# zhongzisha/multi_frame_super_resolution

Hardware: AMD Instinct MI355X
Metric: Mpix/s end-to-end (N-frame burst -> x2 SR) (higher is better)
Workload: dtype f32

## Files before the change

multi_frame_super_resolution_amd/csrc/accumulate_fast.hip:

```cpp
#include <cstdlib>

#include "accumulate_common.hpp"
#include <type_traits>

namespace {

template <int CFA>
struct Cfa {
    static constexpr int col(int yp, int xp) { return (CFA >> (2 * ((yp << 1) | xp))) & 3; }
    static constexpr int pos_of(int c)
    {
        int n = 0, p = -1;
        for (int a = 0; a < 4; a++)
            if (((CFA >> (2 * a)) & 3) == c) {
                n++;
                p = a;
            }
        return n == 1 ? p : -1;
    }
    static constexpr int count(int c)
    {
        int n = 0;
        for (int a = 0; a < 4; a++)
            if (((CFA >> (2 * a)) & 3) == c) n++;
// ... 75 lines not shown
            chS[2] = at_pos(S, pb >> 1, pb & 1);
            chW[2] = at_pos(W, pb >> 1, pb & 1);
        }
        chS[1] = (totS - chS[0]) - chS[2];
        chW[1] = (totW - chW[0]) - chW[2];
    }
#pragma unroll
    for (int c = 0; c < 3; c++) {
        accP[3 * K + c] = __builtin_fmaf(__builtin_fmaf(-lv.black[c], chW[c], chS[c]), lv.invWhite[c], accP[3 * K + c]);
        accW[3 * K + c] += chW[c];
    }
}

__device__ __forceinline__ void tap_weights13(float kx, float ky, float kz, float (&w)[13])
{
    const float a1 = kx * -0.72134752044448170368f, b1 = ky * -0.72134752044448170368f;
    const float c1 = kz * -0.72134752044448170368f;
    const float A[3] = {0.0f, a1, 4.0f * a1}, B[3] = {0.0f, b1, 4.0f * b1};
#pragma unroll
    for (int n = 0; n < 12; n++) {
        const int py = n / 5 - 2, px = n % 5 - 2;
        const int apx = px < 0 ? -px : px, apy = py < 0 ? -py : py;
        const float d = apx == 0 ? B[apy] : (apy == 0 ? A[apx] : A[apx] + B[apy]);
        w[n] = __builtin_amdgcn_exp2f(px * py == 0 ? d : d + (float)(2 * px * py) * c1);
    }
    w[12] = 1.0f;
}

template <int K, int CFA>
__device__ __forceinline__ void strip_pixel_sites(const float (&C)[5][3], const float (&s)[3][3], uint32_t mby, uint32_t nby, uint32_t mP,
                                                   uint32_t mQ, const StripLevels& lv, float* accP, float* accW)
{
    auto andm = [](uint32_t m, float a) { return __uint_as_float(m & __float_as_uint(a)); };
    float Om[3][3];
#pragma unroll
    for (int i = 0; i < 3; i++) {
        Om[0][i] = C[0][i] + andm(nby, C[1][i]);
        Om[1][i] = C[2][i] + selm(mby, C[1][i], C[3][i]);
        Om[2][i] = andm(mby, C[3][i]) + C[4][i];
    }
    float S[2][2], W[2][2];
    S[0][0] = __builtin_fmaf(s[2][2], Om[2][2], __builtin_fmaf(s[2][0], Om[2][0], __builtin_fmaf(s[0][2], Om[0][2], s[0][0] * Om[0][0])));
    W[0][0] = (Om[0][0] + Om[0][2]) + (Om[2][0] + Om[2][2]);
    S[0][1] = __builtin_fmaf(s[2][1], Om[2][1], s[0][1] * Om[0][1]);
    W[0][1] = Om[0][1] + Om[2][1];
    S[1][0] = __builtin_fmaf(s[1][2], Om[1][2], s[1][0] * Om[1][0]);
    W[1][0] = Om[1][0] + Om[1][2];
    S[1][1] = s[1][1] * Om[1][1];
    W[1][1] = Om[1][1];

    classes_to_channels<K, CFA>(S, W, mP, mQ, lv, accP, accW);
}

template <int K, int CFA, bool PARITY = false, typename RawF, typename MaskF>
__device__ __forceinline__ void strip_pixel_w(int X, int Y, int sx, int sy, const float (&w)[13], RawF rawf, MaskF mval,
                                               const StripLevels& lv, float* accP, float* accW)
{
    const int qx = X + sx - 2, qy = Y + sy - 2;
    const int x0 = qx >> 1, y0 = qy >> 1;
    uint32_t mbx = 0u - (uint32_t)(qx & 1), mby = 0u - (uint32_t)(qy & 1);
    uint32_t nbx = ~mbx, nby = ~mby;
    asm volatile("" : "+v"(mbx), "+v"(nbx), "+v"(mby), "+v"(nby));
    const uint32_t mP = 0u - (uint32_t)(x0 & 1), mQ = 0u - (uint32_t)(y0 & 1);
    auto andm = [](uint32_t m, float a) { return __uint_as_float(m & __float_as_uint(a)); };

    float s[3][3];
    rawf(x0, y0, s);

    float wl[13], wh[13];
#pragma unroll
    for (int n = 0; n < 13; n++) {
        const int it = n % 5;
        if (it == 1 || it == 3) {
            wl[n] = andm(nbx, w[n]);
            wh[n] = andm(mbx, w[n]);
        }
    }
    auto W_ = [&](int jt, int it) { const int n = jt * 5 + it; return w[n <= 12 ? n : 24 - n]; };
    auto WL = [&](int jt, int it) { const int n = jt * 5 + it; return wl[n <= 12 ? n : 24 - n]; };
    auto WH = [&](int jt, int it) { const int n = jt * 5 + it; return wh[n <= 12 ? n : 24 - n]; };

    const uint32_t mY13 = mQ ^ mby;
    constexpr int cellLo = (K + 0 + 2) >> 2;
    auto cidx = [](int it) { return (((K + it + 2) >> 2) == ((K + 2) >> 2)) ? 0 : 1; };

    float C[5][3];
#pragma unroll
    for (int jt = 0; jt < 5; jt++) {
        uint32_t mya;
        if (jt == 0 || jt == 4) mya = mQ;
        if (jt == 2) mya = ~mQ;
        if (jt == 1) mya = mY13;
        if (jt == 3) mya = ~mY13;
        float Ee[2], Eo[2];
        if constexpr (PARITY) {
            const int eQ = ((qy << 2) & 8) | ((qx + qx) & 4);
            const int by2 = (qy << 3) & 8;
            const int e = (jt == 0 || jt == 4) ? eQ : (jt == 2 ? (eQ ^ 8) : (jt == 1 ? (eQ ^ by2) : (eQ ^ 8 ^ by2)));
#pragma unroll
            for (int c = 0; c < 2; c++) {
                Ee[c] = mval(jt, cellLo + c, e);
                Eo[c] = mval(jt, cellLo + c, e ^ 4);
            }
        } else {
#pragma unroll
            for (int c = 0; c < 2; c++) {
                float m[3];
#pragma unroll
                for (int ch = 0; ch < 3; ch++) m[ch] = mval(jt, cellLo + c, ch);
                resolve_certainty<CFA>(mya, mP, m, Ee[c], Eo[c]);
            }
        }
        C[jt][0] = cidx(0) == cidx(1) ? (W_(jt, 0) + WL(jt, 1)) * Ee[cidx(0)]
                                      : __builtin_fmaf(WL(jt, 1), Ee[cidx(1)], W_(jt, 0) * Ee[cidx(0)]);
        {
            float acc;
            if (cidx(1) == cidx(2))
                acc = (WH(jt, 1) + W_(jt, 2)) * Eo[cidx(1)];
            else
                acc = __builtin_fmaf(W_(jt, 2), Eo[cidx(2)], WH(jt, 1) * Eo[cidx(1)]);
            if (cidx(3) == cidx(1) && cidx(1) == cidx(2))
                acc = ((WH(jt, 1) + W_(jt, 2)) + WL(jt, 3)) * Eo[cidx(1)];
            else
                acc = __builtin_fmaf(WL(jt, 3), Eo[cidx(3)], acc);
            C[jt][1] = acc;
        }
        C[jt][2] = cidx(3) == cidx(4) ? (WH(jt, 3) + W_(jt, 4)) * Ee[cidx(3)]
                                      : __builtin_fmaf(W_(jt, 4), Ee[cidx(4)], WH(jt, 3) * Ee[cidx(3)]);
    }
    strip_pixel_sites<K, CFA>(C, s, mby, nby, mP, mQ, lv, accP, accW);
}

template <int K, int CFA, typename RawF>
__device__ __forceinline__ void strip_pixel_sat(int X, int Y, int sx, int sy, const float (&w)[13], const float (&P)[3][4], RawF rawf,
                                                 const StripLevels& lv, float* accP, float* accW)
{
    const int qx = X + sx - 2, qy = Y + sy - 2;
    const int x0 = qx >> 1, y0 = qy >> 1;
    uint32_t mbx = 0u - (uint32_t)(qx & 1), mby = 0u - (uint32_t)(qy & 1);
    uint32_t nby = ~mby;
    asm volatile("" : "+v"(mbx), "+v"(mby), "+v"(nby));
    const uint32_t mP = 0u - (uint32_t)(x0 & 1), mQ = 0u - (uint32_t)(y0 & 1);
    float s[3][3];
    rawf(x0, y0, s);
    auto W_ = [&](int jt, int it) { const int n = jt * 5 + it; return w[n <= 12 ? n : 24 - n]; };
    auto P_ = [&](int jt, int i) { return jt <= 2 ? P[jt][i] : P[4 - jt][3 - i]; };
    float C[5][3];
#pragma unroll
    for (int jt = 0; jt < 5; jt++) {
        C[jt][0] = selm(mbx, W_(jt, 0), P_(jt, 0));
        C[jt][1] = selm(mbx, P_(jt, 1), P_(jt, 2));
        C[jt][2] = selm(mbx, P_(jt, 3), W_(jt, 4));
    }
    strip_pixel_sites<K, CFA>(C, s, mby, nby, mP, mQ, lv, accP, accW);
}

__device__ __forceinline__ void tap_pair_sums(const float (&w)[13], float (&P)[3][4])
{
    auto W_ = [&](int jt, int it) { const int n = jt * 5 + it; return w[n <= 12 ? n : 24 - n]; };
#pragma unroll
    for (int r = 0; r < 3; r++)
#pragma unroll
        for (int i = 0; i < 4; i++) P[r][i] = W_(r, i) + W_(r, i + 1);
}

template <int K, int CFA, bool PARITY = false, typename MaskF>
__device__ __forceinline__ void strip_pixel(int X, int Y, int sx, int sy, float kx, float ky, float kz,
                                             const uint16_t* __restrict__ raw, int dimX, MaskF mval,
                                             const StripLevels& lv, float* accP, float* accW)
{
    float w[13];
    tap_weights13(kx, ky, kz, w);
    auto rawf = [&](int x0, int y0, float (&s)[3][3]) {
        const uint16_t* r = raw + (size_t)y0 * dimX + x0;
#pragma unroll
        for (int j = 0; j < 3; j++)
#pragma unroll
            for (int i = 0; i < 3; i++) s[j][i] = (float)r[j * dimX + i];
    };
    strip_pixel_w<K, CFA, PARITY>(X, Y, sx, sy, w, rawf, mval, lv, accP, accW);
}

#define STRIP_MARGIN 16
#ifndef MARGIN_TAP_SUMS
#define MARGIN_TAP_SUMS 1
#endif

template <int SCALE, bool WIN = false>
__global__ void __launch_bounds__(256)
    k_accumulateMargin(const uint16_t* __restrict__ raw, pix3* __restrict__ imgOut, pix3* __restrict__ totalWeights,
                       const float4* __restrict__ certaintyMask, mfsr_tex2d kernelParam, mfsr_tex2d shifts, Levels3 glv,
                       int dimX, int dimY, int strideOut, int strideMask, int cfaPacked, int rowBegin, int rowEnd, MarginRects mr)
{
    constexpr int scale = SCALE;
    if constexpr (WIN) {
        int x, y;
        if (!margin_rect_pixel(mr, blockIdx.x * blockDim.x + threadIdx.x, x, y)) return;
        accumulate_pixel_generic<GEOM_FULL, true, MARGIN_TAP_SUMS>(x, y, raw, imgOut, totalWeights, certaintyMask, kernelParam, shifts,
                                                                   glv, dimX, dimY, scale, strideOut, strideMask, cfaPacked,
                                                                   mr.accX0, mr.accY0);
        return;
    }
    const int hrW = scale * dimX, hrH = scale * dimY, M = STRIP_MARGIN;
    const int rowLen = hrW - 2;
    const int nTop = (M - 1) * rowLen;
    const int nBot = (M - 1) * rowLen;
    const int sideLen = 2 * (M - 1);
    const int nSide = (hrH - 2 * M) * sideLen;
    const int idx = blockIdx.x * blockDim.x + threadIdx.x;
    int x, y;
    if (idx < nTop) {
        y = 1 + idx / rowLen;
        x = 1 + idx % rowLen;
    } else if (idx < nTop + nBot) {
        const int r = idx - nTop;
        y = hrH - M + r / rowLen;
        x = 1 + r % rowLen;
    } else if (idx < nTop + nBot + nSide) {
        const int r = idx - nTop - nBot;
        y = M + r / sideLen;
        const int c = r % sideLen;
        x = c < M - 1 ? 1 + c : hrW - M + (c - (M - 1));
    } else {
        return;
    }
    if (y < rowBegin || y >= rowEnd) return;
    accumulate_pixel_generic<GEOM_FULL, true, MARGIN_TAP_SUMS>(x, y, raw, imgOut, totalWeights, certaintyMask, kernelParam, shifts, glv, dimX,
                                              dimY, scale, strideOut, strideMask, cfaPacked);
}

struct TileFrame {
    const uint16_t* raw;
    const float4* mask;
// ... 195 lines not shown
    const int Y = (blockIdx.y + rowBlock0) * 4 + threadIdx.y;
    const int hrW = 2 * dimX, hrH = 2 * dimY;
    const int X0 = 4 * tx;
    if (X0 < STRIP_MARGIN || X0 >= hrW - STRIP_MARGIN || Y < STRIP_MARGIN || Y >= hrH - STRIP_MARGIN) return;
    if (WIN && (X0 < wx0 || X0 >= wx1)) return;

    const size_t accOff = WIN ? (size_t)(Y - wy0) * strideOut + (size_t)(X0 - wx0) * 12 : (size_t)Y * strideOut + (size_t)X0 * 12;
    float4* pP = (float4*)((char*)imgOut + accOff);
    float4* pW = (float4*)((char*)totalWeights + accOff);
    float accP[12], accW[12];
    {
        const float4 a0 = pP[0], a1 = pP[1], a2 = pP[2];
        const float4 b0 = pW[0], b1 = pW[1], b2 = pW[2];
        accP[0] = a0.x; accP[1] = a0.y; accP[2] = a0.z; accP[3] = a0.w;
        accP[4] = a1.x; accP[5] = a1.y; accP[6] = a1.z; accP[7] = a1.w;
        accP[8] = a2.x; accP[9] = a2.y; accP[10] = a2.z; accP[11] = a2.w;
        accW[0] = b0.x; accW[1] = b0.y; accW[2] = b0.z; accW[3] = b0.w;
        accW[4] = b1.x; accW[5] = b1.y; accW[6] = b1.z; accW[7] = b1.w;
        accW[8] = b2.x; accW[9] = b2.y; accW[10] = b2.z; accW[11] = b2.w;
    }
#pragma unroll
    for (int n = 0; n < NF; n++)
        strip_frame<CFA, FR>(tx, Y, X0, fr.f[n].raw, fr.f[n].mask, kernelParam, fr.f[n].shifts, glv, lv, dimX, dimY, strideMask,
                             cfaPacked, accP, accW);
    pP[0] = make_float4(accP[0], accP[1], accP[2], accP[3]);
    pP[1] = make_float4(accP[4], accP[5], accP[6], accP[7]);
    pP[2] = make_float4(accP[8], accP[9], accP[10], accP[11]);
    pW[0] = make_float4(accW[0], accW[1], accW[2], accW[3]);
    pW[1] = make_float4(accW[4], accW[5], accW[6], accW[7]);
    pW[2] = make_float4(accW[8], accW[9], accW[10], accW[11]);
}

#define TILE_COLS 66
#ifndef TILE_WAVES
#define TILE_WAVES 4
#endif
#ifndef TILE_WAVES2
#define TILE_WAVES2 4
#endif
#ifndef TILE_GROUP_BOTH_PLANES
#define TILE_GROUP_BOTH_PLANES 1
#endif
#define TILE_WAVES_NF(NF) ((NF) == 1 ? TILE_WAVES : ((NF) > 2 && TILE_GROUP_BOTH_PLANES) ? (TILE_LDS_ALIAS_ON ? 4 : 3) : TILE_WAVES2)
#ifndef TILE_PIXEL_MAJOR
#define TILE_PIXEL_MAJOR 1
#endif
#define TILE_LDS_ALIAS_ON (TILE_LDS_ALIAS && TILE_PIXEL_MAJOR && TILE_GROUP_BOTH_PLANES)
#ifndef TILE_LDS_ALIAS
#define TILE_LDS_ALIAS 1
#endif
#ifndef TILE_SAT_PATH
#define TILE_SAT_PATH 1
#endif

template <int CFA, int NF, int FR = 4, bool WIN = false>
__global__ void __launch_bounds__(256, (FR != 4 ? 3 : TILE_WAVES_NF(NF)))
    k_accumulate2xTile(TileFrames<NF> fr, pix3* __restrict__ imgOut, pix3* __restrict__ totalWeights, mfsr_tex2d kernelParam,
                       Levels3 glv, StripLevels lv, int dimX, int dimY, int strideOut, int strideMask, int cfaPacked,
                       int tilesX, int tilesY, int tilesPerXcd, int fresh, int tileY0, int tileX0, int wx0, int wx1, int wy0)
{
    const int pid = (int)blockIdx.x;
    const int tile = tilesPerXcd > 0 ? (pid & 7) * tilesPerXcd + (pid >> 3) : pid;
    if (tile >= tilesX * tilesY) return;
    const int bIdYrel = tile / tilesX, bIdX = tile - bIdYrel * tilesX + (WIN ? tileX0 : 0);
    const int bIdY = bIdYrel + tileY0;
    static_assert(FR == 4 || FR == 2, "field resolution");
    constexpr int FC = 256 / FR + 2, FROWS = 4 / FR + 2;
    constexpr int PL = (NF <= 2 || TILE_GROUP_BOTH_PLANES) ? 2 : 1;
    constexpr bool ALIAS = TILE_LDS_ALIAS_ON && FR == 4 && NF > 2 && PL == 2;
    __shared__ __attribute__((aligned(16))) float4 sAcc[PL][4][192];
    __shared__ float4 sKown[ALIAS ? 1 : FROWS][ALIAS ? 1 : FC];
    __shared__ float2 sFown[ALIAS ? 1 : NF][ALIAS ? 1 : FROWS][ALIAS ? 1 : FC];
    static_assert(!ALIAS || sizeof(float4) * FROWS * FC + sizeof(float2) * NF * FROWS * FC <= sizeof(float4) * 4 * 192, "field texels fit a plane-set");
    float4(*sK)[FC] = ALIAS ? (float4(*)[FC]) & sAcc[PL - 1][0][0] : (float4(*)[FC]) & sKown[0][0];
    float2(*sF)[FROWS][FC] = ALIAS ? (float2(*)[FROWS][FC])((char*)&sAcc[PL - 1][0][0] + sizeof(float4) * FROWS * FC)
                                   : (float2(*)[FROWS][FC]) & sFown[0][0][0];
    __shared__ float4 sM[NF][3][TILE_COLS];
    __shared__ uint32_t sUnsat[3][TILE_COLS];
    __shared__ __attribute__((aligned(16))) float sColA[256];
    __shared__ float sRowB[4];
    const int lx = threadIdx.x, ly = threadIdx.y;
    const int tx = bIdX * 64 + lx;
    const int Y = bIdY * 4 + ly;
    const int hrW = 2 * dimX, hrH = 2 * dimY;
    const int X0 = 4 * tx;
    const int fw = kernelParam.width, fh = kernelParam.height;
    const int mw = dimX / 2, mh = dimY / 2;
    {
        const int t = ly * 64 + lx;
        if constexpr (FR != 4) {
            for (int i = t; i < FROWS * FC; i += 256) {
                const int r = i / FC, c = i - r * FC;
                const int gy = bIdY * (4 / FR) - 1 + r, gx = bIdX * (256 / FR) - 1 + c;
                const int fy = clampi(gy, 0, fh - 1), fx = clampi(gx, 0, fw - 1);
                float4 k = row_ptr((const float4*)kernelParam.ptr, kernelParam.pitch, fy)[fx];
                k.w = psd_ok(k.x, k.y, k.z) ? 1.0f : 0.0f;
                sK[r][c] = k;
#pragma unroll
                for (int n = 0; n < NF; n++) sF[n][r][c] = row_ptr((const float2*)fr.f[n].shifts.ptr, fr.f[n].shifts.pitch, fy)[fx];
            }
            if (t < 3 * TILE_COLS) {
                const int r = t / TILE_COLS, c = t - r * TILE_COLS;
                const int gy = bIdY - 1 + r, gx = bIdX * 64 - 1 + c;
                uint32_t unsat = 0;
#pragma unroll
                for (int n = 0; n < NF; n++) {
                    const float4 m = row_ptr(fr.f[n].mask, strideMask, clampi(gy, 0, mh - 1))[clampi(gx, 0, mw - 1)];
                    const float mc[3] = {sane(m.x), sane(m.y), sane(m.z)};
                    sM[n][r][c] = make_float4(mc[Cfa<CFA>::col(0, 0)], mc[Cfa<CFA>::col(0, 1)], mc[Cfa<CFA>::col(1, 0)],
                                              mc[Cfa<CFA>::col(1, 1)]);
                    if (!(mc[0] == 1.0f && mc[1] == 1.0f && mc[2] == 1.0f)) unsat |= 1u << n;
                }
                sUnsat[r][c] = unsat;
            }
        } else if (t < 3 * TILE_COLS) {
            const int r = t / TILE_COLS, c = t - r * TILE_COLS;
            const int gy = bIdY - 1 + r, gx = bIdX * 64 - 1 + c;
            const int fy = clampi(gy, 0, fh - 1), fx = clampi(gx, 0, fw - 1);
            float4 k = row_ptr((const float4*)kernelParam.ptr, kernelParam.pitch, fy)[fx];
            k.w = psd_ok(k.x, k.y, k.z) ? 1.0f : 0.0f;
            sK[r][c] = k;
            uint32_t unsat = 0;
#pragma unroll
            for (int n = 0; n < NF; n++) {
                sF[n][r][c] = row_ptr((const float2*)fr.f[n].shifts.ptr, fr.f[n].shifts.pitch, fy)[fx];
                const float4 m = row_ptr(fr.f[n].mask, strideMask, clampi(gy, 0, mh - 1))[clampi(gx, 0, mw - 1)];
                const float mc[3] = {sane(m.x), sane(m.y), sane(m.z)};
                sM[n][r][c] = make_float4(mc[Cfa<CFA>::col(0, 0)], mc[Cfa<CFA>::col(0, 1)], mc[Cfa<CFA>::col(1, 0)],
                                          mc[Cfa<CFA>::col(1, 1)]);
                if (!(mc[0] == 1.0f && mc[1] == 1.0f && mc[2] == 1.0f)) unsat |= 1u << n;
            }
            sUnsat[r][c] = unsat;
        }
        {
            const int X = bIdX * 256 + t;
            const float posX = ((float)X + 0.5f) / (float)hrW;
            float xB = posX * (float)fw - 0.5f;
            if (!finitef(xB)) xB = 0.0f;
            const float fxf = floorf(xB);
            const int txc = FR == 4 ? X >> 2 : X >> 1, ci = FR == 4 ? ((t & 3) < 2 ? 0 : 1) : (t & 1);
            const bool ok = (f2i(fxf) == txc - 1 + ci) && (txc + ci <= fw - 1);
            sColA[t] = ok ? xB - fxf : -1.0f;
        }
        if (t < 4) {
            const int Yr = bIdY * 4 + t;
            const float posY = ((float)Yr + 0.5f) / (float)hrH;
            float yB = posY * (float)fh - 0.5f;
            if (!finitef(yB)) yB = 0.0f;
            const float fyf = floorf(yB);
            const int frr = FR == 4 ? (t < 2 ? 0 : 1) : (t + 1) >> 1;
            const bool ok = (f2i(fyf) == bIdY * (4 / FR) - 1 + frr) && f2i(fyf) >= 0 && f2i(fyf) + 1 <= fh - 1;
            sRowB[t] = ok ? yB - fyf : -1.0f;
        }
    }
    const bool rowLive = Y >= STRIP_MARGIN && Y < hrH - STRIP_MARGIN;
    const size_t rowBytes = (size_t)hrW * 12;
    const size_t segByte = (size_t)bIdX * 3072;
    const size_t winB0 = WIN ? (size_t)wx0 * 12 : 0, winB1 = WIN ? (size_t)wx1 * 12 : 0;
    char* gP = WIN ? (char*)imgOut + (size_t)(Y - wy0) * strideOut : (char*)imgOut + (size_t)Y * strideOut + segByte;
    char* gW = WIN ? (char*)totalWeights + (size_t)(Y - wy0) * strideOut : (char*)totalWeights + (size_t)Y * strideOut + segByte;
    auto inWin = [&](size_t gb) { return !WIN || (gb >= winB0 && gb + 16 <= winB1); };
    auto chunk = [&](char* g, size_t off) { return WIN ? g + (segByte + off - winB0) : g + off; };
    auto stage_plane = [&](char* g, int pl) {
#pragma unroll
        for (int j = 0; j < 3; j++) {
            if (fresh) {
                sAcc[pl][ly][j * 64 + lx] = make_float4(0.0f, 0.0f, 0.0f, 0.0f);
            } else {
                const size_t off = (size_t)(j * 64 + lx) * 16;
                if (segByte + off + 16 <= rowBytes && inWin(segByte + off))
                    __builtin_amdgcn_global_load_lds((const __attribute__((address_space(1))) void*)chunk(g, off),
                                                     (__attribute__((address_space(3))) void*)&sAcc[pl][ly][j * 64], 16, 0, 0);
            }
        }
    };
    if (rowLive) {
        stage_plane(gP, 0);
        if (PL == 2 && !ALIAS) stage_plane(gW, 1);
    }
    __syncthreads();
    if (!rowLive) return;
    const bool stripLive = X0 >= STRIP_MARGIN && X0 < hrW - STRIP_MARGIN;
// ... 13 lines not shown
        float4 Kt[2][SC];
#pragma unroll
        for (int r = 0; r < 2; r++)
#pragma unroll
            for (int c = 0; c < SC; c++) Kt[r][c] = sK[fr_ + r][cb + c];
        float kAll = ((Kt[0][0].w * Kt[0][1].w) * (Kt[0][2].w * Kt[1][0].w)) * (Kt[1][1].w * Kt[1][2].w);
        if (SC == 4) kAll *= Kt[0][SC - 1].w * Kt[1][SC - 1].w;
        kOk = kAll > 0.0f;
#pragma unroll
        for (int k = 0; k < 4; k++) {
            const int ci = ciOf(k);
            const float w00 = (1.0f - av[k]) * (1.0f - b), w10 = av[k] * (1.0f - b), w01 = (1.0f - av[k]) * b, w11 = av[k] * b;
            auto mix = [&](float t00, float t10, float t01, float t11) {
                return __builtin_fmaf(w11, t11, __builtin_fmaf(w01, t01, __builtin_fmaf(w10, t10, w00 * t00)));
            };
            kxa[k] = mix(Kt[0][ci].x, Kt[0][ci + 1].x, Kt[1][ci].x, Kt[1][ci + 1].x);
            kya[k] = mix(Kt[0][ci].y, Kt[0][ci + 1].y, Kt[1][ci].y, Kt[1][ci + 1].y);
            kza[k] = mix(Kt[0][ci].z, Kt[0][ci + 1].z, Kt[1][ci].z, Kt[1][ci + 1].z);
        }
    }

    float accP[12], accW[12];
#pragma unroll
    for (int i = 0; i < 12; i++) accP[i] = accW[i] = 0.0f;
    const uint32_t xmax = (uint32_t)(2 * dimX - 5), ymax = (uint32_t)(2 * dimY - 5);
    uint32_t safeBits = 0;
    static_assert(NF <= 2 || TILE_PIXEL_MAJOR, "three and four frames per launch exist in pixel-major order only");
#if TILE_PIXEL_MAJOR
    if constexpr (NF > 1 || FR != 4) {
        uint32_t sxy[NF][ALIAS ? 2 : 4];
        int bsx[NF], bsy[NF];
#pragma unroll
        for (int n = 0; n < NF; n++) {
            bsx[n] = bsy[n] = 0;
            if constexpr (ALIAS) {
                sxy[n][0] = sxy[n][1] = 0u;
                const float2 cf = sF[n][1][FC / 2];
                bsx[n] = __builtin_amdgcn_readfirstlane(min(max(round2i(cf.x * 2.0f), -32000), 32000));
                bsy[n] = __builtin_amdgcn_readfirstlane(min(max(round2i(cf.y * 2.0f), -32000), 32000));
            }
            float2 Ft[2][SC];
#pragma unroll
            for (int r = 0; r < 2; r++)
#pragma unroll
                for (int c = 0; c < SC; c++) Ft[r][c] = sF[n][fr_ + r][cb + c];
            bool safe = geomOk && kOk;
#pragma unroll
            for (int k = 0; k < 4; k++) {
                const int ci = ciOf(k);
                const float ux = lerp4(Ft[0][ci].x, Ft[0][ci + 1].x, Ft[1][ci].x, Ft[1][ci + 1].x, av[k], b);
                const float uy = lerp4(Ft[0][ci].y, Ft[0][ci + 1].y, Ft[1][ci].y, Ft[1][ci + 1].y, av[k], b);
                const int sx = round2i(ux * 2.0f), sy = round2i(uy * 2.0f);
                const int qx = X0 + k + sx - 2, qy = Y + sy - 2;
                safe = safe && (uint32_t)(sx + (1 << 15)) < (2u << 15) && (uint32_t)(sy + (1 << 15)) < (2u << 15) &&
                       (uint32_t)qx <= xmax && (uint32_t)qy <= ymax;
                if constexpr (ALIAS) {
                    const int dx = sx - bsx[n], dy = sy - bsy[n];
                    safe = safe && (uint32_t)(dx + 128) < 256u && (uint32_t)(dy + 128) < 256u;
                    sxy[n][0] |= ((uint32_t)dx & 0xffu) << (8 * k);
                    sxy[n][1] |= ((uint32_t)dy & 0xffu) << (8 * k);
                } else {
                    sxy[n][k] = ((uint32_t)sx & 0xffffu) | ((uint32_t)sy << 16);
                }
            }
            if (safe) safeBits |= 1u << n;
        }
        if constexpr (ALIAS) {
            __syncthreads();
            stage_plane(gW, 1);
        }
        const float* mrow[5];
#pragma unroll
        for (int jt = 0; jt < 5; jt++) mrow[jt] = (const float*)&sM[0][((ly + jt - 2) >> 2) + 1][lx];
        const char* rawRow[NF][3];
#pragma unroll
        for (int n = 0; n < NF; n++)
#pragma unroll
            for (int j = 0; j < 3; j++) rawRow[n][j] = (const char*)(fr.f[n].raw + (size_t)j * dimX);
        uint32_t satW = 0;
        if constexpr (TILE_SAT_PATH) {
            const int r0 = ((ly - 2) >> 2) + 1;
            uint32_t u = sUnsat[r0][lx] | sUnsat[r0 + 1][lx];
            if (lx < 2) u |= sUnsat[r0][64 + lx] | sUnsat[r0 + 1][64 + lx];
#pragma unroll
            for (int n = 0; n < NF; n++)
                if (__builtin_amdgcn_ballot_w64((u >> n) & 1u) == 0) satW |= 1u << n;
            satW = (uint32_t)__builtin_amdgcn_readfirstlane((int)satW);
        }
        auto pixel = [&](auto kc) {
            constexpr int k = decltype(kc)::value;
            if (safeBits == 0) return;
            float aP[12];
            aP[3 * k] = aP[3 * k + 1] = aP[3 * k + 2] = 0.0f;
            float w[13];
            tap_weights13(kxa[k], kya[k], kza[k], w);
            float P[3][4];
            if (TILE_SAT_PATH && satW) tap_pair_sums(w, P);
#pragma unroll
            for (int n = 0; n < NF; n++) {
                if ((safeBits >> n) & 1u) {
                    auto rawf = [&](int x0, int y0, float (&sv)[3][3]) {
                        const uint32_t boff = (uint32_t)(y0 * dimX + x0) * 2u;
#pragma unroll
                        for (int j = 0; j < 3; j++) {
                            const char* rb = rawRow[n][j] + (size_t)boff;
#pragma unroll
                            for (int i = 0; i < 3; i++) sv[j][i] = (float)*(const uint16_t*)(rb + 2 * i);
                        }
                    };
                    auto mval = [&](int jt, int cell, int e4) {
                        return *(const float*)((const char*)(mrow[jt] + n * (3 * TILE_COLS * 4) + cell * 4) + e4);
                    };
                    const int sx = ALIAS ? bsx[n] + (int)(int8_t)(sxy[n][0] >> (8 * k)) : (int)(int16_t)(sxy[n][ALIAS ? 0 : k] & 0xffffu);
                    const int sy = ALIAS ? bsy[n] + (int)(int8_t)(sxy[n][1] >> (8 * k)) : (int)sxy[n][ALIAS ? 0 : k] >> 16;
                    if (TILE_SAT_PATH && ((satW >> n) & 1u))
                        strip_pixel_sat<k, CFA>(X0 + k, Y, sx, sy, w, P, rawf, lv, aP, accW);
                    else
                        strip_pixel_w<k, CFA, true>(X0 + k, Y, sx, sy, w, rawf, mval, lv, aP, accW);
                }
            }
            if (k == 0) asm volatile("s_waitcnt vmcnt(0)" ::: "memory");
            float* myP = (float*)&sAcc[0][ly][0] + lx * 12 + 3 * k;
            myP[0] += aP[3 * k];
            myP[1] += aP[3 * k + 1];
            myP[2] += aP[3 * k + 2];
        };
        pixel(std::integral_constant<int, 0>{});
        pixel(std::integral_constant<int, 1>{});
        pixel(std::integral_constant<int, 2>{});
        pixel(std::integral_constant<int, 3>{});
    } else
#endif
    {
#pragma unroll 1
    for (int n = 0; n < NF; n++) {
        const uint16_t* raw = (NF > 1 && n) ? fr.f[NF - 1].raw : fr.f[0].raw;
        float avn[4] = {av[0], av[1], av[2], av[3]};
        float bn = b;
#pragma unroll
        for (int k = 0; k < 4; k++) asm volatile("" : "+v"(avn[k]));
        asm volatile("" : "+v"(bn));
#define av avn
#define b bn
        float2 Ft[2][3];
#pragma unroll
        for (int r = 0; r < 2; r++)
#pragma unroll
            for (int c = 0; c < 3; c++) Ft[r][c] = sF[n][fr_ + r][lx + c];
        int sx[4], sy[4];
        bool safe = geomOk && kOk;
#pragma unroll
        for (int k = 0; k < 4; k++) {
            const int ci = k < 2 ? 0 : 1;
            const float ux = lerp4(Ft[0][ci].x, Ft[0][ci + 1].x, Ft[1][ci].x, Ft[1][ci + 1].x, av[k], b);
            const float uy = lerp4(Ft[0][ci].y, Ft[0][ci + 1].y, Ft[1][ci].y, Ft[1][ci + 1].y, av[k], b);
            sx[k] = round2i(ux * 2.0f);
            sy[k] = round2i(uy * 2.0f);
            const int qx = X0 + k + sx[k] - 2, qy = Y + sy[k] - 2;
            safe = safe && (uint32_t)(sx[k] + (1 << 20)) < (2u << 20) && (uint32_t)(sy[k] + (1 << 20)) < (2u << 20) &&
                   (uint32_t)qx <= xmax && (uint32_t)qy <= ymax;
        }
#undef av
#undef b
        if (safe) {
            safeBits |= 1u << n;
#pragma unroll
            for (int k = 0; k < 4; k++) asm volatile("" : "+v"(kxa[k]), "+v"(kya[k]), "+v"(kza[k]));
            auto mval = [&](int jt, int cell, int e4) {
                const int mr = ((ly + jt - 2) >> 2) + 1;
                return *(const float*)((const char*)&sM[n][mr][lx + cell] + e4);
            };
            strip_pixel<0, CFA, true>(X0 + 0, Y, sx[0], sy[0], kxa[0], kya[0], kza[0], raw, dimX, mval, lv, accP, accW);
            strip_pixel<1, CFA, true>(X0 + 1, Y, sx[1], sy[1], kxa[1], kya[1], kza[1], raw, dimX, mval, lv, accP, accW);
            strip_pixel<2, CFA, true>(X0 + 2, Y, sx[2], sy[2], kxa[2], kya[2], kza[2], raw, dimX, mval, lv, accP, accW);
            strip_pixel<3, CFA, true>(X0 + 3, Y, sx[3], sy[3], kxa[3], kya[3], kza[3], raw, dimX, mval, lv, accP, accW);
        }
    }
    }
    auto add_plane = [&](int pl, const float* acc) {
        float4* my = (float4*)((float*)&sAcc[pl][ly][0] + lx * 12);
#pragma unroll
        for (int j = 0; j < 3; j++) {
            float4 a = my[j];
            a.x += acc[4 * j + 0]; a.y += acc[4 * j + 1]; a.z += acc[4 * j + 2]; a.w += acc[4 * j + 3];
            my[j] = a;
        }
    };
    auto slow_frames = [&](auto doP, auto doW, int plP, int plW) {
        constexpr bool DO_P = decltype(doP)::value, DO_W = decltype(doW)::value;
        float* myP = (float*)&sAcc[plP][ly][0] + lx * 12;
        float* myW = (float*)&sAcc[plW][ly][0] + lx * 12;
#pragma unroll 1
        for (int n = 0; n < NF; n++) {
            if (!((safeBits >> n) & 1u) && stripLive) {
                TileFrame F = fr.f[0];
#pragma unroll
                for (int m = 1; m < NF; m++)
                    if (n == m) F = fr.f[m];
#pragma unroll 1
                for (int k = 0; k < 4; k++) {
                    const int X = X0 + k;
                    if (X >= 1 && X < hrW - 1) {
                        pix3 px = {0.0f, 0.0f, 0.0f}, tw = {0.0f, 0.0f, 0.0f};
                        if (DO_P) px = {myP[3 * k], myP[3 * k + 1], myP[3 * k + 2]};
                        if (DO_W) tw = {myW[3 * k], myW[3 * k + 1], myW[3 * k + 2]};
                        accumulate_pixel_core<GEOM_FULL, true>(X, Y, F.raw, F.mask, kernelParam, F.shifts, glv, dimX, dimY, 2,
                                                               strideMask, cfaPacked, px, tw);
                        if (DO_P) { myP[3 * k] = px.x; myP[3 * k + 1] = px.y; myP[3 * k + 2] = px.z; }
                        if (DO_W) { myW[3 * k] = tw.x; myW[3 * k + 1] = tw.y; myW[3 * k + 2] = tw.z; }
                    }
                }
            }
        }
    };
    auto store_plane = [&](int pl, char* g) {
        asm volatile("s_waitcnt lgkmcnt(0)" ::: "memory");
#pragma unroll
        for (int j = 0; j < 3; j++) {
            const size_t off = (size_t)(j * 64 + lx) * 16;
            const size_t gb = segByte + off;
            const bool sideMargin = gb < (size_t)STRIP_MARGIN * 12 || gb + 16 > rowBytes - (size_t)STRIP_MARGIN * 12;
            if (gb + 16 <= rowBytes && (fresh || !sideMargin) && inWin(gb)) *(float4*)chunk(g, off) = sAcc[pl][ly][j * 64 + lx];
        }
    };
    using Yes = std::true_type;
    using No = std::false_type;
    asm volatile("s_waitcnt vmcnt(0)" ::: "memory");
    constexpr bool valueSumsStaged = TILE_PIXEL_MAJOR && (NF > 1 || FR != 4);
// ... 387 lines not shown
    if (safeBits) {
#pragma unroll
        for (int j = 0; j < 3; j++) {
            float4 a = ((float4*)myP)[j], c = ((float4*)myW)[j];
            a.x += accP[4 * j + 0]; a.y += accP[4 * j + 1]; a.z += accP[4 * j + 2]; a.w += accP[4 * j + 3];
            c.x += accW[4 * j + 0]; c.y += accW[4 * j + 1]; c.z += accW[4 * j + 2]; c.w += accW[4 * j + 3];
            ((float4*)myP)[j] = a;
            ((float4*)myW)[j] = c;
        }
    }
#pragma unroll 1
    for (int n = 0; n < NF; n++) {
        TileFrame F = fr.f[0];
#pragma unroll
        for (int m = 1; m < NF; m++)
            if (n == m) F = fr.f[m];
        if (!((safeBits >> n) & 1u) && stripLive) {
#pragma unroll 1
            for (int k = 0; k < 4; k++) {
                const int X = X0 + k;
                if (X >= 1 && X < hrW - 1) {
                    pix3 px = {myP[3 * k], myP[3 * k + 1], myP[3 * k + 2]};
                    pix3 tw = {myW[3 * k], myW[3 * k + 1], myW[3 * k + 2]};
                    accumulate_pixel_core<GEOM_FULL, true>(X, Y, F.raw, F.mask, kernelParam, F.shifts, glv, dimX, dimY, 4,
                                                           strideMask, cfaPacked, px, tw);
                    myP[3 * k] = px.x; myP[3 * k + 1] = px.y; myP[3 * k + 2] = px.z;
                    myW[3 * k] = tw.x; myW[3 * k + 1] = tw.y; myW[3 * k + 2] = tw.z;
                }
            }
        }
    }
    __syncthreads();
#pragma unroll
    for (int j = 0; j < 3; j++) {
        const size_t off = (size_t)(j * 64 + lx) * 16;
        const size_t g = segByte + off;
        const bool sideMargin = g < (size_t)STRIP_MARGIN * 12 || g + 16 > rowBytes - (size_t)STRIP_MARGIN * 12;
        if (g + 16 <= rowBytes && (fresh || !sideMargin) && inWin(g)) {
            *(float4*)chunk(gP, off) = sAcc[0][r][h * 192 + j * 64 + lx];
            *(float4*)chunk(gW, off) = sAcc[1][r][h * 192 + j * 64 + lx];
        }
    }
}

constexpr int pack_cfa(int c00, int c01, int c10, int c11) { return c00 | (c01 << 2) | (c10 << 4) | (c11 << 6); }

int g_strip_xcd_remap = 1;
int g_strip_use_tile = 1;

bool tile_kernel_ok(mfsr_tex2d kp, mfsr_tex2d sh, int dimX, int dimY)
{
    const int hrW = 2 * dimX, hrH = 2 * dimY;
    return kp.width == sh.width && kp.height == sh.height && kp.width * 4 == hrW && kp.height * 4 == hrH && kp.width >= 4 &&
           (dimX % 4) == 0 && (dimY % 4) == 0 && g_strip_use_tile == 1;
}

bool tile_kernel_ok_fr2(mfsr_tex2d kp, mfsr_tex2d sh, int dimX, int dimY)
{
    const int hrW = 2 * dimX, hrH = 2 * dimY;
    return kp.width == sh.width && kp.height == sh.height && kp.width * 2 == hrW && kp.height * 2 == hrH && kp.width >= 4 &&
           (dimX % 4) == 0 && (dimY % 4) == 0 && g_strip_use_tile == 1;
}

struct WinLaunch {
    bool on;
    int tileX0, tilesX;
    int x0, x1, y0;
};
WinLaunch win_launch(const HrWindow& w, int hrW, int tileW)
{
    WinLaunch l;
    l.on = w.rel && !(w.x0 == 0 && w.x1 == hrW && w.y0 == 0);
    l.tileX0 = l.on ? w.x0 / tileW : 0;
    l.tilesX = (l.on ? mfsr_cdiv(w.x1, tileW) : mfsr_cdiv(hrW, tileW)) - l.tileX0;
    l.x0 = l.on ? w.x0 : 0;
    l.x1 = l.on ? w.x1 : hrW;
    l.y0 = l.on ? w.y0 : 0;
    return l;
}

template <int CFA, int NF, int FR = 4>
void launch_tile(dim3 grid, dim3 block, hipStream_t st, const TileFrames<NF>& fr, pix3* imgOut, pix3* tw, mfsr_tex2d kp,
                 Levels3 glv, StripLevels lv, int dimX, int dimY, int strideOut, int strideMask, int cfaPacked, int fresh, int tileY0,
                 const WinLaunch& wl)
{
    const int tilesX = (int)grid.x, tilesY = (int)grid.y;
    const int tilesPerXcd = g_strip_xcd_remap ? mfsr_cdiv(tilesX * tilesY, 8) : 0;
    static const int ldsPad = [] {
        const char* e = getenv("MFSR_TILE_LDS_PAD");
        return e ? atoi(e) : 0;
    }();
    const dim3 g1(tilesPerXcd ? 8 * tilesPerXcd : tilesX * tilesY);
    if (wl.on)
        hipLaunchKernelGGL((k_accumulate2xTile<CFA, NF, FR, true>), g1, block, ldsPad, st, fr, imgOut, tw, kp, glv, lv, dimX, dimY,
                           strideOut, strideMask, cfaPacked, tilesX, tilesY, tilesPerXcd, fresh, tileY0, wl.tileX0, wl.x0, wl.x1, wl.y0);
    else
        hipLaunchKernelGGL((k_accumulate2xTile<CFA, NF, FR>), g1, block, ldsPad, st, fr, imgOut, tw, kp, glv, lv, dimX, dimY,
                           strideOut, strideMask, cfaPacked, tilesX, tilesY, tilesPerXcd, fresh, tileY0, 0, 0, 0, 0);
}

template <int CFA, int FR, int NF>
void launch_strip_regs_fr(dim3 grid, dim3 block, hipStream_t st, const TileFrames<NF>& fr, pix3* imgOut, pix3* tw, mfsr_tex2d kp,
                          Levels3 glv, StripLevels lv, int dimX, int dimY, int strideOut, int strideMask, int cfaPacked, int rowBlock0,
                          const WinLaunch& wl)
{
    if (wl.on)
        hipLaunchKernelGGL((k_accumulate2xStrip<CFA, FR, NF, true>), grid, block, 0, st, fr, imgOut, tw, kp, glv, lv, dimX, dimY,
                           strideOut, strideMask, cfaPacked, rowBlock0, wl.tileX0, wl.x0, wl.x1, wl.y0);
    else
        hipLaunchKernelGGL((k_accumulate2xStrip<CFA, FR, NF>), grid, block, 0, st, fr, imgOut, tw, kp, glv, lv, dimX, dimY,
                           strideOut, strideMask, cfaPacked, rowBlock0, 0, 0, 0, 0);
}

template <int CFA, int NF>
// ... 354 lines not shown
```

Measured before the change: 22680.

## Store certainty mask as per-CFA-position LDS planes and use 32-bit raw offsets

The staged certainty mask in LDS moves from an array of float4 per cell to four separate planes indexed by CFA position. The strip-pixel mask lookup now adds precomputed plane and row byte offsets held in 32-bit LDS addresses instead of deriving the parity offset per tap. Raw frame reads switch to a scalar base pointer plus a 32-bit per-lane offset to cut 64-bit address arithmetic, and the tile-kernel eligibility checks are tightened so raw images must fit 32-bit byte offsets. The sx/sy range check is also skipped on the alias path, since the 8-bit delta check already bounds those values.

```diff
diff --git a/multi_frame_super_resolution_amd/csrc/accumulate_fast.hip b/multi_frame_super_resolution_amd/csrc/accumulate_fast.hip
--- a/multi_frame_super_resolution_amd/csrc/accumulate_fast.hip
+++ b/multi_frame_super_resolution_amd/csrc/accumulate_fast.hip
@@ -151,10 +151,11 @@
     classes_to_channels<K, CFA>(S, W, mP, mQ, lv, accP, accW);
 }
 
-template <int K, int CFA, bool PARITY = false, typename RawF, typename MaskF>
+template <int K, int CFA, int EP = 0, typename RawF, typename MaskF>
 __device__ __forceinline__ void strip_pixel_w(int X, int Y, int sx, int sy, const float (&w)[13], RawF rawf, MaskF mval,
                                                const StripLevels& lv, float* accP, float* accW)
 {
+    static_assert(EP == 0 || EP >= 4, "EP: 0 (by channel), 4 (texels by CFA position) or the plane stride in bytes");
     const int qx = X + sx - 2, qy = Y + sy - 2;
     const int x0 = qx >> 1, y0 = qy >> 1;
     uint32_t mbx = 0u - (uint32_t)(qx & 1), mby = 0u - (uint32_t)(qy & 1);
@@ -183,6 +184,15 @@
     constexpr int cellLo = (K + 0 + 2) >> 2;
     auto cidx = [](int it) { return (((K + it + 2) >> 2) == ((K + 2) >> 2)) ? 0 : 1; };
 
+    uint32_t ex[2] = {0u, 0u}, ey[4] = {0u, 0u, 0u, 0u};
+    if constexpr (EP > 4) {
+        ex[0] = mP & (uint32_t)EP;
+        ex[1] = ex[0] ^ (uint32_t)EP;
+        ey[0] = mQ & (uint32_t)(2 * EP);
+        ey[1] = ey[0] ^ (uint32_t)(2 * EP);
+        ey[2] = mY13 & (uint32_t)(2 * EP);
+        ey[3] = ey[2] ^ (uint32_t)(2 * EP);
+    }
     float C[5][3];
 #pragma unroll
     for (int jt = 0; jt < 5; jt++) {
@@ -192,7 +202,14 @@
         if (jt == 1) mya = mY13;
         if (jt == 3) mya = ~mY13;
         float Ee[2], Eo[2];
-        if constexpr (PARITY) {
+        if constexpr (EP > 4) {
+            const uint32_t eyj = ey[(jt == 0 || jt == 4) ? 0 : (jt == 2 ? 1 : (jt == 1 ? 2 : 3))];
+#pragma unroll
+            for (int c = 0; c < 2; c++) {
+                Ee[c] = mval(jt, cellLo + c, eyj, ex[0]);
+                Eo[c] = mval(jt, cellLo + c, eyj, ex[1]);
+            }
+        } else if constexpr (EP == 4) {
             const int eQ = ((qy << 2) & 8) | ((qx + qx) & 4);
             const int by2 = (qy << 3) & 8;
             const int e = (jt == 0 || jt == 4) ? eQ : (jt == 2 ? (eQ ^ 8) : (jt == 1 ? (eQ ^ by2) : (eQ ^ 8 ^ by2)));
@@ -263,7 +280,7 @@
         for (int i = 0; i < 4; i++) P[r][i] = W_(r, i) + W_(r, i + 1);
 }
 
-template <int K, int CFA, bool PARITY = false, typename MaskF>
+template <int K, int CFA, int EP = 0, typename MaskF>
 __device__ __forceinline__ void strip_pixel(int X, int Y, int sx, int sy, float kx, float ky, float kz,
                                              const uint16_t* __restrict__ raw, int dimX, MaskF mval,
                                              const StripLevels& lv, float* accP, float* accW)
@@ -277,7 +294,7 @@
 #pragma unroll
             for (int i = 0; i < 3; i++) s[j][i] = (float)r[j * dimX + i];
     };
-    strip_pixel_w<K, CFA, PARITY>(X, Y, sx, sy, w, rawf, mval, lv, accP, accW);
+    strip_pixel_w<K, CFA, EP>(X, Y, sx, sy, w, rawf, mval, lv, accP, accW);
 }
 
 #define STRIP_MARGIN 16
@@ -579,6 +596,18 @@
 #ifndef TILE_SAT_PATH
 #define TILE_SAT_PATH 1
 #endif
+#ifndef TILE_CERT_PLANES
+#define TILE_CERT_PLANES 1
+#endif
+#ifndef TILE_RAW_LANE32
+#define TILE_RAW_LANE32 1
+#endif
+#ifndef TILE_ALIAS_IMPLIED
+#define TILE_ALIAS_IMPLIED 1
+#endif
+#ifndef TILE_LEVELS_VGPR
+#define TILE_LEVELS_VGPR 0
+#endif
 
 template <int CFA, int NF, int FR = 4, bool WIN = false>
 __global__ void __launch_bounds__(256, (FR != 4 ? 3 : TILE_WAVES_NF(NF)))
@@ -603,6 +632,18 @@
     float2(*sF)[FROWS][FC] = ALIAS ? (float2(*)[FROWS][FC])((char*)&sAcc[PL - 1][0][0] + sizeof(float4) * FROWS * FC)
                                    : (float2(*)[FROWS][FC]) & sFown[0][0][0];
     __shared__ float4 sM[NF][3][TILE_COLS];
+    float(*sMp)[3][NF][TILE_COLS] = (float(*)[3][NF][TILE_COLS]) & sM[0][0][0];
+    constexpr int EP = TILE_CERT_PLANES ? 3 * NF * TILE_COLS * 4 : 4;
+    auto stage_cert = [&](int n, int r, int c, const float (&mc)[3]) {
+        if constexpr (TILE_CERT_PLANES) {
+            sMp[0][r][n][c] = mc[Cfa<CFA>::col(0, 0)];
+            sMp[1][r][n][c] = mc[Cfa<CFA>::col(0, 1)];
+            sMp[2][r][n][c] = mc[Cfa<CFA>::col(1, 0)];
+            sMp[3][r][n][c] = mc[Cfa<CFA>::col(1, 1)];
+        } else {
+            sM[n][r][c] = make_float4(mc[Cfa<CFA>::col(0, 0)], mc[Cfa<CFA>::col(0, 1)], mc[Cfa<CFA>::col(1, 0)], mc[Cfa<CFA>::col(1, 1)]);
+        }
+    };
     __shared__ uint32_t sUnsat[3][TILE_COLS];
     __shared__ __attribute__((aligned(16))) float sColA[256];
     __shared__ float sRowB[4];
@@ -634,8 +675,7 @@
                 for (int n = 0; n < NF; n++) {
                     const float4 m = row_ptr(fr.f[n].mask, strideMask, clampi(gy, 0, mh - 1))[clampi(gx, 0, mw - 1)];
                     const float mc[3] = {sane(m.x), sane(m.y), sane(m.z)};
-                    sM[n][r][c] = make_float4(mc[Cfa<CFA>::col(0, 0)], mc[Cfa<CFA>::col(0, 1)], mc[Cfa<CFA>::col(1, 0)],
-                                              mc[Cfa<CFA>::col(1, 1)]);
+                    stage_cert(n, r, c, mc);
                     if (!(mc[0] == 1.0f && mc[1] == 1.0f && mc[2] == 1.0f)) unsat |= 1u << n;
                 }
                 sUnsat[r][c] = unsat;
@@ -653,8 +693,7 @@
                 sF[n][r][c] = row_ptr((const float2*)fr.f[n].shifts.ptr, fr.f[n].shifts.pitch, fy)[fx];
                 const float4 m = row_ptr(fr.f[n].mask, strideMask, clampi(gy, 0, mh - 1))[clampi(gx, 0, mw - 1)];
                 const float mc[3] = {sane(m.x), sane(m.y), sane(m.z)};
-                sM[n][r][c] = make_float4(mc[Cfa<CFA>::col(0, 0)], mc[Cfa<CFA>::col(0, 1)], mc[Cfa<CFA>::col(1, 0)],
-                                          mc[Cfa<CFA>::col(1, 1)]);
+                stage_cert(n, r, c, mc);
                 if (!(mc[0] == 1.0f && mc[1] == 1.0f && mc[2] == 1.0f)) unsat |= 1u << n;
             }
             sUnsat[r][c] = unsat;
@@ -774,13 +813,14 @@
                 const float uy = lerp4(Ft[0][ci].y, Ft[0][ci + 1].y, Ft[1][ci].y, Ft[1][ci + 1].y, av[k], b);
                 const int sx = round2i(ux * 2.0f), sy = round2i(uy * 2.0f);
                 const int qx = X0 + k + sx - 2, qy = Y + sy - 2;
-                safe = safe && (uint32_t)(sx + (1 << 15)) < (2u << 15) && (uint32_t)(sy + (1 << 15)) < (2u << 15) &&
-                       (uint32_t)qx <= xmax && (uint32_t)qy <= ymax;
+                if constexpr (!(ALIAS && TILE_ALIAS_IMPLIED))
+                    safe = safe && (uint32_t)(sx + (1 << 15)) < (2u << 15) && (uint32_t)(sy + (1 << 15)) < (2u << 15);
+                safe = safe && (uint32_t)qx <= xmax && (uint32_t)qy <= ymax;
                 if constexpr (ALIAS) {
-                    const int dx = sx - bsx[n], dy = sy - bsy[n];
-                    safe = safe && (uint32_t)(dx + 128) < 256u && (uint32_t)(dy + 128) < 256u;
-                    sxy[n][0] |= ((uint32_t)dx & 0xffu) << (8 * k);
-                    sxy[n][1] |= ((uint32_t)dy & 0xffu) << (8 * k);
+                    const uint32_t dx = (uint32_t)sx - (uint32_t)bsx[n], dy = (uint32_t)sy - (uint32_t)bsy[n];
+                    safe = safe && dx + 128u < 256u && dy + 128u < 256u;
+                    sxy[n][0] |= (dx & 0xffu) << (8 * k);
+                    sxy[n][1] |= (dy & 0xffu) << (8 * k);
                 } else {
                     sxy[n][k] = ((uint32_t)sx & 0xffffu) | ((uint32_t)sy << 16);
                 }
@@ -791,14 +831,37 @@
             __syncthreads();
             stage_plane(gW, 1);
         }
-        const float* mrow[5];
-#pragma unroll
-        for (int jt = 0; jt < 5; jt++) mrow[jt] = (const float*)&sM[0][((ly + jt - 2) >> 2) + 1][lx];
-        const char* rawRow[NF][3];
-#pragma unroll
-        for (int n = 0; n < NF; n++)
-#pragma unroll
-            for (int j = 0; j < 3; j++) rawRow[n][j] = (const char*)(fr.f[n].raw + (size_t)j * dimX);
+        typedef const __attribute__((address_space(3))) char* lds_cptr;
+        const float* mrow[5] = {};
+        uint32_t mrowA[5] = {};
+#pragma unroll
+        for (int jt = 0; jt < 5; jt++) {
+            if constexpr (TILE_CERT_PLANES) {
+                mrowA[jt] = (uint32_t)(uintptr_t)(lds_cptr)&sMp[0][((ly + jt - 2) >> 2) + 1][0][lx];
+                asm volatile("" : "+v"(mrowA[jt]));
+            } else {
+                mrow[jt] = (const float*)&sM[0][((ly + jt - 2) >> 2) + 1][lx];
+            }
+        }
+        typedef const __attribute__((address_space(1))) char* glb_cptr;
+        const char* rawRow[NF][3] = {};
+        glb_cptr rawBase[NF] = {};
+        const uint32_t rawPitch = (uint32_t)dimX * 2u;
+#pragma unroll
+        for (int n = 0; n < NF; n++) {
+            if constexpr (TILE_RAW_LANE32) {
+                rawBase[n] = (glb_cptr)fr.f[n].raw;
+                asm volatile("" : "+s"(rawBase[n]));
+            } else {
+#pragma unroll
+                for (int j = 0; j < 3; j++) rawRow[n][j] = (const char*)(fr.f[n].raw + (size_t)j * dimX);
+            }
+        }
+        StripLevels lvv = lv;
+        if constexpr (TILE_LEVELS_VGPR) {
+#pragma unroll
+            for (int c = 0; c < 3; c++) asm volatile("" : "+v"(lvv.black[c]), "+v"(lvv.invWhite[c]));
+        }
         uint32_t satW = 0;
         if constexpr (TILE_SAT_PATH) {
             const int r0 = ((ly - 2) >> 2) + 1;
@@ -825,20 +888,33 @@
                         const uint32_t boff = (uint32_t)(y0 * dimX + x0) * 2u;
 #pragma unroll
                         for (int j = 0; j < 3; j++) {
-                            const char* rb = rawRow[n][j] + (size_t)boff;
-#pragma unroll
-                            for (int i = 0; i < 3; i++) sv[j][i] = (float)*(const uint16_t*)(rb + 2 * i);
+                            if constexpr (TILE_RAW_LANE32) {
+                                uint32_t off = boff + (uint32_t)j * rawPitch;
+                                asm volatile("" : "+v"(off));
+                                glb_cptr rb = rawBase[n] + off;
+#pragma unroll
+                                for (int i = 0; i < 3; i++)
+                                    sv[j][i] = (float)*(const __attribute__((address_space(1))) uint16_t*)(rb + 2 * i);
+                            } else {
+                                const char* rb = rawRow[n][j] + (size_t)boff;
+#pragma unroll
+                                for (int i = 0; i < 3; i++) sv[j][i] = (float)*(const uint16_t*)(rb + 2 * i);
+                            }
                         }
                     };
-                    auto mval = [&](int jt, int cell, int e4) {
-                        return *(const float*)((const char*)(mrow[jt] + n * (3 * TILE_COLS * 4) + cell * 4) + e4);
+                    auto mval = [&](int jt, int cell, auto... e) {
+                        if constexpr (TILE_CERT_PLANES)
+                            return *(const __attribute__((address_space(3))) float*)(uintptr_t)((mrowA[jt] + ... + e) +
+                                                                                                 (uint32_t)(n * TILE_COLS + cell) * 4u);
+                        else
+                            return *(const float*)((const char*)(mrow[jt] + n * (3 * TILE_COLS * 4) + cell * 4) + (e + ...));
                     };
                     const int sx = ALIAS ? bsx[n] + (int)(int8_t)(sxy[n][0] >> (8 * k)) : (int)(int16_t)(sxy[n][ALIAS ? 0 : k] & 0xffffu);
                     const int sy = ALIAS ? bsy[n] + (int)(int8_t)(sxy[n][1] >> (8 * k)) : (int)sxy[n][ALIAS ? 0 : k] >> 16;
                     if (TILE_SAT_PATH && ((satW >> n) & 1u))
-                        strip_pixel_sat<k, CFA>(X0 + k, Y, sx, sy, w, P, rawf, lv, aP, accW);
+                        strip_pixel_sat<k, CFA>(X0 + k, Y, sx, sy, w, P, rawf, lvv, aP, accW);
                     else
-                        strip_pixel_w<k, CFA, true>(X0 + k, Y, sx, sy, w, rawf, mval, lv, aP, accW);
+                        strip_pixel_w<k, CFA, EP>(X0 + k, Y, sx, sy, w, rawf, mval, lvv, aP, accW);
                 }
             }
             if (k == 0) asm volatile("s_waitcnt vmcnt(0)" ::: "memory");
@@ -888,14 +964,17 @@
             safeBits |= 1u << n;
 #pragma unroll
             for (int k = 0; k < 4; k++) asm volatile("" : "+v"(kxa[k]), "+v"(kya[k]), "+v"(kza[k]));
-            auto mval = [&](int jt, int cell, int e4) {
+            auto mval = [&](int jt, int cell, auto... e) {
                 const int mr = ((ly + jt - 2) >> 2) + 1;
-                return *(const float*)((const char*)&sM[n][mr][lx + cell] + e4);
+                if constexpr (TILE_CERT_PLANES)
+                    return *(const float*)((const char*)&sMp[0][mr][n][lx + cell] + (e + ...));
+                else
+                    return *(const float*)((const char*)&sM[n][mr][lx + cell] + (e + ...));
             };
-            strip_pixel<0, CFA, true>(X0 + 0, Y, sx[0], sy[0], kxa[0], kya[0], kza[0], raw, dimX, mval, lv, accP, accW);
-            strip_pixel<1, CFA, true>(X0 + 1, Y, sx[1], sy[1], kxa[1], kya[1], kza[1], raw, dimX, mval, lv, accP, accW);
-            strip_pixel<2, CFA, true>(X0 + 2, Y, sx[2], sy[2], kxa[2], kya[2], kza[2], raw, dimX, mval, lv, accP, accW);
-            strip_pixel<3, CFA, true>(X0 + 3, Y, sx[3], sy[3], kxa[3], kya[3], kza[3], raw, dimX, mval, lv, accP, accW);
+            strip_pixel<0, CFA, EP>(X0 + 0, Y, sx[0], sy[0], kxa[0], kya[0], kza[0], raw, dimX, mval, lv, accP, accW);
+            strip_pixel<1, CFA, EP>(X0 + 1, Y, sx[1], sy[1], kxa[1], kya[1], kza[1], raw, dimX, mval, lv, accP, accW);
+            strip_pixel<2, CFA, EP>(X0 + 2, Y, sx[2], sy[2], kxa[2], kya[2], kza[2], raw, dimX, mval, lv, accP, accW);
+            strip_pixel<3, CFA, EP>(X0 + 3, Y, sx[3], sy[3], kxa[3], kya[3], kza[3], raw, dimX, mval, lv, accP, accW);
         }
     }
     }
@@ -1389,14 +1468,14 @@
 {
     const int hrW = 2 * dimX, hrH = 2 * dimY;
     return kp.width == sh.width && kp.height == sh.height && kp.width * 4 == hrW && kp.height * 4 == hrH && kp.width >= 4 &&
-           (dimX % 4) == 0 && (dimY % 4) == 0 && g_strip_use_tile == 1;
+           (dimX % 4) == 0 && (dimY % 4) == 0 && (uint64_t)dimX * (uint64_t)dimY * 2u < (1ull << 32) && g_strip_use_tile == 1;
 }
 
 bool tile_kernel_ok_fr2(mfsr_tex2d kp, mfsr_tex2d sh, int dimX, int dimY)
 {
     const int hrW = 2 * dimX, hrH = 2 * dimY;
     return kp.width == sh.width && kp.height == sh.height && kp.width * 2 == hrW && kp.height * 2 == hrH && kp.width >= 4 &&
-           (dimX % 4) == 0 && (dimY % 4) == 0 && g_strip_use_tile == 1;
+           (dimX % 4) == 0 && (dimY % 4) == 0 && (uint64_t)dimX * (uint64_t)dimY * 2u < (1ull << 32) && g_strip_use_tile == 1;
 }
 
 struct WinLaunch {
```

Result: faster. 23270 (median of 6 runs) (+2.6%).
